# callmeray/PointMVSNet

Hardware: AMD Instinct MI355X
Metric: depth-maps/sec (DTU 640x512, 3 src views, 2 flow iters) (higher is better)
Workload: dtype f32

## Files before the change

### pointmvsnet_amd/csrc/conv3d.hip

```cpp
#include <stdlib.h>

#include "pf_common.h"
#include "pf_bn_resolve.h"

namespace {

typedef float f32x4 __attribute__((ext_vector_type(4)));

struct ConvGeom {
  int Cin, Cout, Di, Hi, Wi, Do, Ho, Wo;
  int ID, IH, IW, IWP, plane;
  int tiles_d, tiles_h, tiles_w;
  int aff_mode, sps, aff_off;
  const float* in_scale;
  const float* in_shift;
  pf_bn_job in_bn;
};

template <int STRIDE, int TD>
struct Stage {
  static constexpr int ID = (TD - 1) * STRIDE + 3;
  static constexpr int IH = 3 * STRIDE + 3;
  static constexpr int IW = 15 * STRIDE + 3;
  static constexpr int IWP = IW + 1;
  static constexpr int RAW = ID * IH * IWP;
  static constexpr int WANT = STRIDE == 1 ? 16 : 17;
  static constexpr int PLANE = RAW + ((WANT - RAW % 32) + 32) % 32;
  static constexpr int ELEMS = ID * IH * IW;
  static constexpr int NXR = (ELEMS + 63) / 64;
};

template <int NT, int STRIDE, int TD, int MINW>
__global__ __launch_bounds__(256, MINW) void conv3d_k3_kernel(const float* __restrict__ x, const float* __restrict__ wp,
                                                        float* __restrict__ y, ConvGeom g,
                                                        double* __restrict__ partials) {
  using St = Stage<STRIDE, TD>;
  constexpr int ID = St::ID, IH = St::IH, IW = St::IW, IWP = St::IWP, PLANE = St::PLANE;
  constexpr int ELEMS = St::ELEMS, NXR = St::NXR;
  constexpr int NCP = NT * 16;
  constexpr int WSZ = 27 * 4 * NCP;
  constexpr int NWR = (WSZ + 255) / 256;
  constexpr int XS = 4 * PLANE;
  extern __shared__ __attribute__((aligned(16))) float lds[];
  float* xs0 = lds;
  float* ws0 = lds + 2 * XS;
  float* tile = lds;
  double* red = reinterpret_cast<double*>(tile + 4 * NCP * 17 + ((4 * NCP * 17) & 1));

  const int tid = threadIdx.x;
  const int wave = __builtin_amdgcn_readfirstlane(tid >> 6), lane = tid & 63;
  const int li = lane & 15, lk = lane >> 4;
  unsigned xb_, xn_;
  pf_xcd_xy<PF_XCD_CONV3D>(xb_, xn_);
  const int n = (int)xn_, bx = (int)xb_;
  const int plane_i = g.Hi * g.Wi, vol_i = plane_i * g.Di;
  const int64_t plane_o = (int64_t)g.Ho * g.Wo, vol_o = plane_o * g.Do;
  const float* xb = x + (int64_t)n * g.Cin * vol_i;
  float* yb = y + (int64_t)n * g.Cout * vol_o;
  const int cgroups = g.Cin >> 2;

  double ssum[NT], ssq[NT];
#pragma unroll
  for (int t = 0; t < NT; ++t) ssum[t] = ssq[t] = 0.0;

  float* aff = lds + g.aff_off;
  if (g.aff_mode == 1) {
    const int stat = n / g.sps;
    for (int e = tid; e < 2 * g.Cin; e += 256)
      aff[e] = e < g.Cin ? g.in_scale[(int64_t)stat * g.Cin + e] : g.in_shift[(int64_t)stat * g.Cin + e - g.Cin];
  } else if (g.aff_mode == 2) {
    pf_bn_resolve<256>(g.in_bn, n / g.sps, aff, aff + g.Cin, reinterpret_cast<double*>(lds));
  }

  const int total = g.tiles_d * g.tiles_h * g.tiles_w;
  for (int item = bx; item < total; item += gridDim.x) {
    const int tw = item % g.tiles_w;
    const int rest = item / g.tiles_w;
    const int th = rest % g.tiles_h;
    const int td = rest / g.tiles_h;
    const int od0 = td * TD, oh0 = th * 4, ow0 = tw * 16;
    const int id0 = od0 * STRIDE - 1, ih0 = oh0 * STRIDE - 1, iw0 = ow0 * STRIDE - 1;

    unsigned gofs[NXR];
    unsigned okmask = 0;
#pragma unroll
    for (int r = 0; r < NXR; ++r) {
      const int e = lane + 64 * r;
      const int row = e / IW, col = e - row * IW;
      const int dz = row / IH, hy = row - dz * IH;
      const int id = id0 + dz, ih = ih0 + hy, iw = iw0 + col;
      const bool ok = e < ELEMS && id >= 0 && id < g.Di && ih >= 0 && ih < g.Hi && iw >= 0 && iw < g.Wi;
      gofs[r] = ok ? (unsigned)(id * plane_i + ih * g.Wi + iw) : 0u;
      okmask |= (ok ? 1u : 0u) << r;
    }

    float rx[NXR], rw[NWR];
    auto load_group = [&](int cg) {
      const float* src = xb + (int64_t)(cg * 4 + wave) * vol_i;
#pragma unroll
      for (int r = 0; r < NXR; ++r) rx[r] = src[gofs[r]];
      const float* wsrc = wp + (int64_t)cg * WSZ;
#pragma unroll
      for (int r = 0; r < NWR; ++r) {
        const int e = tid + 256 * r;
        rw[r] = (256 * (r + 1) <= WSZ || e < WSZ) ? wsrc[e] : 0.0f;
      }
    };
    auto store_group = [&](int buf, int cg) {
      float* xs = xs0 + buf * XS + wave * PLANE;
      float* ws = ws0 + buf * WSZ;
      float sa = 1.0f, sb = 0.0f;
      if (g.aff_mode) {
        sa = aff[cg * 4 + wave];
        sb = aff[g.Cin + cg * 4 + wave];
      }
#pragma unroll
      for (int r = 0; r < NXR; ++r) {
        const int e = lane + 64 * r;
        float v = rx[r];
        if (g.aff_mode) v = fmaxf(fmaf(v, sa, sb), 0.0f);
        if (64 * (r + 1) <= ELEMS || e < ELEMS) xs[e + e / IW] = ((okmask >> r) & 1u) ? v : 0.0f;
      }
#pragma unroll
      for (int r = 0; r < NWR; ++r) {
        const int e = tid + 256 * r;
        if (256 * (r + 1) <= WSZ || e < WSZ) ws[e] = rw[r];
      }
    };

    f32x4 acc[TD][NT];
#pragma unroll
    for (int d = 0; d < TD; ++d)
#pragma unroll
      for (int t = 0; t < NT; ++t) acc[d][t] = (f32x4){0.0f, 0.0f, 0.0f, 0.0f};

    __syncthreads();
    load_group(0);
    store_group(0, 0);
    __syncthreads();
    for (int cg = 0; cg < cgroups; ++cg) {
      const int buf = cg & 1;
      if (cg + 1 < cgroups) load_group(cg + 1);
      const float* xs = xs0 + buf * XS + lk * PLANE + (wave * STRIDE) * IWP + li * STRIDE;
      const float* ws = ws0 + buf * WSZ + lk * NCP + li;
#pragma unroll
      for (int kd = 0; kd < 3; ++kd) {
#pragma unroll
        for (int kh = 0; kh < 3; ++kh) {
#pragma unroll
          for (int kw = 0; kw < 3; ++kw) {
            const int tap = (kd * 3 + kh) * 3 + kw;
            float b[NT];
#pragma unroll
            for (int t = 0; t < NT; ++t) b[t] = ws[tap * 4 * NCP + 16 * t];
#pragma unroll
            for (int d = 0; d < TD; ++d) {
              const float a = xs[((d * STRIDE + kd) * IH + kh) * IWP + kw];
#pragma unroll
              for (int t = 0; t < NT; ++t) acc[d][t] = __builtin_amdgcn_mfma_f32_16x16x4f32(a, b[t], acc[d][t], 0, 0, 0);
            }
          }
        }
      }
      if (cg + 1 < cgroups) store_group(buf ^ 1, cg + 1);
      __syncthreads();
    }

    const int oh = oh0 + wave;
    float* tl = tile + wave * NCP * 17;
#pragma unroll
    for (int d = 0; d < TD; ++d) {
      const int od = od0 + d;
      const bool row_ok = oh < g.Ho && od < g.Do;
#pragma unroll
      for (int t = 0; t < NT; ++t) {
        float s = 0.0f, q = 0.0f;
#pragma unroll
        for (int r = 0; r < 4; ++r) {
          const int pos = lk * 4 + r;
          const float v = acc[d][t][r];
          tl[(16 * t + li) * 17 + pos] = v;
          if (row_ok && ow0 + pos < g.Wo) {
            s += v;
            q += v * v;
          }
        }
        s += __shfl_xor(s, 16);
        q += __shfl_xor(q, 16);
        s += __shfl_xor(s, 32);
        q += __shfl_xor(q, 32);
        ssum[t] += (double)s;
        ssq[t] += (double)q;
      }
      __builtin_amdgcn_wave_barrier();
      if (row_ok) {
        for (int e = lane; e < NCP * 16; e += 64) {
          const int co = e >> 4, pos = e & 15;
          if (co < g.Cout && ow0 + pos < g.Wo)
            yb[(int64_t)co * vol_o + (int64_t)od * plane_o + (int64_t)oh * g.Wo + ow0 + pos] = tl[co * 17 + pos];
        }
      }
      __builtin_amdgcn_wave_barrier();
    }
  }

  if (partials != nullptr) {
#pragma unroll
    for (int t = 0; t < NT; ++t) {
      if (lane < 16) {
        red[((wave * NCP) + 16 * t + lane) * 2 + 0] = ssum[t];
        red[((wave * NCP) + 16 * t + lane) * 2 + 1] = ssq[t];
      }
    }
    __syncthreads();
    if (tid < g.Cout) {
      double s = 0.0, q = 0.0;
#pragma unroll
      for (int w = 0; w < 4; ++w) {
        s += red[((w * NCP) + tid) * 2 + 0];
        q += red[((w * NCP) + tid) * 2 + 1];
      }
      double* o = partials + (((int64_t)n * gridDim.x + bx) * g.Cout + tid) * 2;
      o[0] = s;
      o[1] = q;
    }
  }
}

template <int COUT>
__global__ __launch_bounds__(256) void conv3d_k3_few_kernel(const float* __restrict__ x, const float* __restrict__ w,
                                                            float* __restrict__ y, int Cin, int D, int H, int W) {
  extern __shared__ __attribute__((aligned(16))) float wl[];
  for (int e = threadIdx.x; e < COUT * Cin * 27; e += 256) wl[e] = w[e];
  __syncthreads();
  const int64_t plane = (int64_t)H * W, vol = plane * D;
  const int64_t i = (int64_t)blockIdx.x * 256 + threadIdx.x;
  const int n = blockIdx.y;
  if (i >= vol) return;
  const int od = (int)(i / plane);
  const int rem = (int)(i - (int64_t)od * plane);
  const int oh = rem / W, ow = rem - oh * W;
  float acc[COUT];
#pragma unroll
  for (int c = 0; c < COUT; ++c) acc[c] = 0.0f;
  const float* xb = x + (int64_t)n * Cin * vol;
  for (int ci = 0; ci < Cin; ++ci) {
    const float* xc = xb + (int64_t)ci * vol;
#pragma unroll
    for (int kd = 0; kd < 3; ++kd) {
      const int id = od + kd - 1;
      const bool dok = id >= 0 && id < D;
#pragma unroll
      for (int kh = 0; kh < 3; ++kh) {
        const int ih = oh + kh - 1;
        const bool hok = dok && ih >= 0 && ih < H;
        const float* row = xc + (int64_t)id * plane + (int64_t)ih * W;
#pragma unroll
        for (int kw = 0; kw < 3; ++kw) {
          const int iw = ow + kw - 1;
          const float v = (hok && iw >= 0 && iw < W) ? row[iw] : 0.0f;
#pragma unroll
          for (int c = 0; c < COUT; ++c) acc[c] = fmaf(v, wl[(c * Cin + ci) * 27 + (kd * 3 + kh) * 3 + kw], acc[c]);
        }
      }
    }
  }
#pragma unroll
  for (int c = 0; c < COUT; ++c) y[((int64_t)n * COUT + c) * vol + i] = acc[c];
}

ConvGeom make_geom(int64_t Cin, int64_t Cout, int64_t Di, int64_t Hi, int64_t Wi, int stride, int td) {
  ConvGeom g;
  g.Cin = (int)Cin;
  g.Cout = (int)Cout;
  g.Di = (int)Di;
  g.Hi = (int)Hi;
  g.Wi = (int)Wi;
  g.Do = (int)((Di - 1) / stride + 1);
  g.Ho = (int)((Hi - 1) / stride + 1);
  g.Wo = (int)((Wi - 1) / stride + 1);
  g.ID = (td - 1) * stride + 3;
  g.IH = 3 * stride + 3;
  g.IW = 15 * stride + 3;
  g.IWP = g.IW + 1;
  const int raw = g.ID * g.IH * g.IWP;
  const int want = stride == 1 ? 16 : 17;
  g.plane = raw + ((want - raw % 32) + 32) % 32;
  g.tiles_d = (g.Do + td - 1) / td;
  g.tiles_h = (g.Ho + 3) / 4;
  g.tiles_w = (g.Wo + 15) / 16;
  g.aff_mode = 0;
  g.sps = 1;
  g.aff_off = 0;
  g.in_scale = g.in_shift = nullptr;
  g.in_bn = pf_bn_job{};
  return g;
}

constexpr size_t kMaxLds = 80 * 1024;

size_t lds_work_bytes(const ConvGeom& g, int NT) {
  const int NCP = NT * 16;
  const size_t staging = sizeof(float) * (size_t)(2 * 4 * g.plane + 2 * 27 * 4 * NCP);
  const size_t epilogue = sizeof(float) * (size_t)(4 * NCP * 17 + 1) + sizeof(double) * (size_t)(4 * NCP * 2);
  const size_t m = staging > epilogue ? staging : epilogue;
  return (m + 15) / 16 * 16;
}
size_t lds_bytes_for(const ConvGeom& g, int NT) {
  return lds_work_bytes(g, NT) + sizeof(float) * 2 * (size_t)g.Cin;
}

int pick_td(int64_t Cin, int64_t Cout, int64_t Di, int64_t Hi, int64_t Wi, int stride) {
  const int NT = (int)((Cout + 15) / 16);
  int best = 0;
  for (int td = (stride == 1 && NT > 1) ? 4 : 2; td >= 1; td >>= 1) {
    const ConvGeom g = make_geom(Cin, Cout, Di, Hi, Wi, stride, td);
    if (lds_bytes_for(g, NT) > kMaxLds) continue;
    best = td;
    if ((int64_t)g.tiles_d * g.tiles_h * g.tiles_w >= 512) return td;
  }
  return best;
}

int blocks_for(const ConvGeom& g) {
  const int64_t total = (int64_t)g.tiles_d * g.tiles_h * g.tiles_w;
#ifndef PF_CONV3D_CAP
#define PF_CONV3D_CAP 2048
#endif
  if (total <= PF_CONV3D_CAP) return (int)total;
  const int64_t per = (total + PF_CONV3D_CAP - 1) / PF_CONV3D_CAP;
  return (int)((total + per - 1) / per);
}

template <int NT, int STRIDE, int TD, int MINW>
int launch(const float* x, const float* wp, float* y, const ConvGeom& g, int64_t N, double* partials,
           hipStream_t s) {
  const size_t lds_bytes = lds_bytes_for(g, NT);
  if (lds_bytes > kMaxLds) return PF_ERR_UNSUPPORTED;
  ConvGeom gk = g;
  gk.aff_off = (int)(lds_work_bytes(g, NT) / sizeof(float));
  if (lds_bytes > 64 * 1024) {
    static std::atomic<unsigned long long> done{0};
    const int rc = pf_allow_big_lds(reinterpret_cast<const void*>(&conv3d_k3_kernel<NT, STRIDE, TD, MINW>),
                                    (int)kMaxLds, done);
    if (rc != PF_OK) return rc;
  }
  dim3 grid((unsigned)blocks_for(g), (unsigned)N);
  hipLaunchKernelGGL((conv3d_k3_kernel<NT, STRIDE, TD, MINW>), grid, dim3(256), lds_bytes, s, x, wp, y, gk, partials);
  return pf_launch_status();
}

template <int NT, int STRIDE, int TD>
int launch_w(const float* x, const float* wp, float* y, const ConvGeom& g, int64_t N, double* partials,
             hipStream_t s) {
  constexpr int kDefault = (NT == 1 && STRIDE == 1 && TD == 2) ? 4 : 2;
  return launch<NT, STRIDE, TD, kDefault>(x, wp, y, g, N, partials, s);
}

template <int NT, int STRIDE>
int launch_td(int td, const float* x, const float* wp, float* y, const ConvGeom& g, int64_t N, double* partials,
              hipStream_t s) {
  if constexpr (STRIDE == 1) {
    if (td == 4) return launch_w<NT, STRIDE, 4>(x, wp, y, g, N, partials, s);
  }
  if (td == 2) return launch_w<NT, STRIDE, 2>(x, wp, y, g, N, partials, s);
  return launch_w<NT, STRIDE, 1>(x, wp, y, g, N, partials, s);
}

}

extern "C" {

int pf_conv3d_blocks(int64_t Cin, int64_t Cout, int64_t Di, int64_t Hi, int64_t Wi, int stride) {
  if (Cin <= 0 || Cout <= 0 || Di <= 0 || Hi <= 0 || Wi <= 0 || (stride != 1 && stride != 2)) return 0;
  const int td = pick_td(Cin, Cout, Di, Hi, Wi, stride);
  if (td == 0) return 0;
  return blocks_for(make_geom(Cin, Cout, Di, Hi, Wi, stride, td));
}

int pf_conv3d_k3_f32(const float* x, const float* wp, float* y, int64_t N, int64_t Cin, int64_t Cout, int64_t Di,
                     int64_t Hi, int64_t Wi, int stride, const float* in_scale, const float* in_shift,
                     const pf_bn_job* in_bn, int samples_per_stat, double* partials, void* stream) {
  PF_REQUIRE(N >= 0 && Cin >= 4 && Cout >= 1 && Di >= 1 && Hi >= 1 && Wi >= 1 && N <= 65535);
  PF_REQUIRE(stride == 1 || stride == 2);
  PF_REQUIRE(samples_per_stat >= 1 && (in_scale == nullptr) == (in_shift == nullptr));
  PF_REQUIRE(in_bn == nullptr || in_scale == nullptr);
  if (in_bn != nullptr && N > 0) {
    PF_REQUIRE(N % samples_per_stat == 0);
    const int rc = pf_bn_in_check(in_bn, (int)Cin, (int)(N / samples_per_stat));
    if (rc != PF_OK) return rc;
  }
  if ((Cin % 4) != 0 || Cout > 32) return PF_ERR_UNSUPPORTED;
  PF_REQUIRE(Cin * Di * Hi * Wi <= INT32_MAX);
  if (N == 0) return PF_OK;
  PF_REQUIRE(x && wp && y);
  const int td = pick_td(Cin, Cout, Di, Hi, Wi, stride);
  if (td == 0) return PF_ERR_UNSUPPORTED;
  ConvGeom g = make_geom(Cin, Cout, Di, Hi, Wi, stride, td);
  g.aff_mode = in_bn ? 2 : (in_scale ? 1 : 0);
  g.sps = samples_per_stat;
  g.in_scale = in_scale;
  g.in_shift = in_shift;
  if (in_bn) g.in_bn = *in_bn;
  hipStream_t s = (hipStream_t)stream;
  const int NT = (int)((Cout + 15) / 16);
  if (stride == 1)
    return NT == 1 ? launch_td<1, 1>(td, x, wp, y, g, N, partials, s) : launch_td<2, 1>(td, x, wp, y, g, N, partials, s);
  return NT == 1 ? launch_td<1, 2>(td, x, wp, y, g, N, partials, s) : launch_td<2, 2>(td, x, wp, y, g, N, partials, s);
}

int pf_conv3d_k3_few_f32(const float* x, const float* w, float* y, int64_t N, int64_t Cin, int64_t Cout, int64_t D,
                         int64_t H, int64_t W, void* stream) {
  PF_REQUIRE(N >= 0 && Cin >= 1 && Cout >= 1 && D >= 1 && H >= 1 && W >= 1 && N <= 65535);
  if (Cout > 4 || Cout * Cin * 27 * sizeof(float) > 48 * 1024) return PF_ERR_UNSUPPORTED;
  PF_REQUIRE(H * W <= INT32_MAX);
  if (N == 0) return PF_OK;
  PF_REQUIRE(x && w && y);
  const size_t lds = sizeof(float) * (size_t)(Cout * Cin * 27);
  dim3 grid((unsigned)pf_cdiv(D * H * W, 256), (unsigned)N);
  hipStream_t s = (hipStream_t)stream;
  switch ((int)Cout) {
    case 1: hipLaunchKernelGGL(conv3d_k3_few_kernel<1>, grid, dim3(256), lds, s, x, w, y, (int)Cin, (int)D, (int)H, (int)W); break;
    case 2: hipLaunchKernelGGL(conv3d_k3_few_kernel<2>, grid, dim3(256), lds, s, x, w, y, (int)Cin, (int)D, (int)H, (int)W); break;
    case 3: hipLaunchKernelGGL(conv3d_k3_few_kernel<3>, grid, dim3(256), lds, s, x, w, y, (int)Cin, (int)D, (int)H, (int)W); break;
    default: hipLaunchKernelGGL(conv3d_k3_few_kernel<4>, grid, dim3(256), lds, s, x, w, y, (int)Cin, (int)D, (int)H, (int)W); break;
  }
  return pf_launch_status();
}

}
```

### pointmvsnet_amd/csrc/conv3d_pair.hip

```cpp
#include <stdlib.h>

#include "pf_common.h"

namespace {

typedef float f32x4 __attribute__((ext_vector_type(4)));

struct PairGeom {
  int Cin, Cout, D, H, W;
  int tiles_d, tiles_h, tiles_w;
};

template <int TD>
struct PStage {
  static constexpr int ID = TD + 2;
  static constexpr int IH = 10;
  static constexpr int IW = 18;
  static constexpr int IWP = IW + 1;
  static constexpr int RAW = ID * IH * IWP;
  static constexpr int PLANE = RAW + ((16 - RAW % 32) + 32) % 32;
  static constexpr int ELEMS = ID * IH * IW;
  static constexpr int NXR = (ELEMS + 63) / 64;
};

constexpr int kTaps = 36;
constexpr int kWsz = kTaps * 4 * 16;

template <int TD>
constexpr size_t pair_lds_bytes() {
  using St = PStage<TD>;
  const size_t staging = sizeof(float) * (size_t)(2 * 4 * St::PLANE + 2 * kWsz);
  const size_t epilogue = sizeof(float) * (size_t)(4 * 16 * 17 + 1) + sizeof(double) * (size_t)(4 * 16 * 2);
  return staging > epilogue ? staging : epilogue;
}

template <int TD, int MINW>
__global__ __launch_bounds__(256, MINW) void conv3d_k3_pair_kernel(const float* __restrict__ x,
                                                                   const float* __restrict__ wp,
                                                                   float* __restrict__ y, PairGeom g,
                                                                   double* __restrict__ partials) {
  using St = PStage<TD>;
  constexpr int ID = St::ID, IH = St::IH, IW = St::IW, IWP = St::IWP, PLANE = St::PLANE;
  constexpr int ELEMS = St::ELEMS, NXR = St::NXR;
  constexpr int NWR = (kWsz + 255) / 256;
  constexpr int XS = 4 * PLANE;
  extern __shared__ __attribute__((aligned(16))) float lds[];
  float* xs0 = lds;
  float* ws0 = lds + 2 * XS;
  float* tile = lds;
  double* red = reinterpret_cast<double*>(tile + 4 * 16 * 17 + ((4 * 16 * 17) & 1));

  const int tid = threadIdx.x;
  const int wave = __builtin_amdgcn_readfirstlane(tid >> 6), lane = tid & 63;
  const int li = lane & 15, lk = lane >> 4;
  unsigned xb_, xn_;
  pf_xcd_xy<PF_XCD_CONV3D>(xb_, xn_);
  const int n = (int)xn_, bx = (int)xb_;
  const int plane_i = g.H * g.W, vol = plane_i * g.D;
  const float* xb = x + (int64_t)n * g.Cin * vol;
  float* yb = y + (int64_t)n * g.Cout * vol;
  const int cgroups = g.Cin >> 2;

  double ssum = 0.0, ssq = 0.0;

  const int total = g.tiles_d * g.tiles_h * g.tiles_w;
  for (int item = bx; item < total; item += gridDim.x) {
    const int tw = item % g.tiles_w;
    const int rest = item / g.tiles_w;
    const int th = rest % g.tiles_h;
    const int td = rest / g.tiles_h;
    const int od0 = td * TD, oh0 = th * 8, ow0 = tw * 16;
    const int id0 = od0 - 1, ih0 = oh0 - 1, iw0 = ow0 - 1;

    unsigned gofs[NXR];
    unsigned okmask = 0;
#pragma unroll
    for (int r = 0; r < NXR; ++r) {
      const int e = lane + 64 * r;
      const int row = e / IW, col = e - row * IW;
      const int dz = row / IH, hy = row - dz * IH;
      const int id = id0 + dz, ih = ih0 + hy, iw = iw0 + col;
      const bool ok = e < ELEMS && id >= 0 && id < g.D && ih >= 0 && ih < g.H && iw >= 0 && iw < g.W;
      gofs[r] = ok ? (unsigned)(id * plane_i + ih * g.W + iw) : 0u;
      okmask |= (ok ? 1u : 0u) << r;
    }

    float rx[NXR], rw[NWR];
    auto load_group = [&](int cg) {
      const float* src = xb + (int64_t)(cg * 4 + wave) * vol;
#pragma unroll
      for (int r = 0; r < NXR; ++r) rx[r] = src[gofs[r]];
      const float* wsrc = wp + (int64_t)cg * kWsz;
#pragma unroll
      for (int r = 0; r < NWR; ++r) {
        const int e = tid + 256 * r;
        rw[r] = (256 * (r + 1) <= kWsz || e < kWsz) ? wsrc[e] : 0.0f;
      }
    };
    auto store_group = [&](int buf) {
      float* xs = xs0 + buf * XS + wave * PLANE;
      float* ws = ws0 + buf * kWsz;
#pragma unroll
      for (int r = 0; r < NXR; ++r) {
        const int e = lane + 64 * r;
        if (64 * (r + 1) <= ELEMS || e < ELEMS) xs[e + e / IW] = ((okmask >> r) & 1u) ? rx[r] : 0.0f;
      }
#pragma unroll
      for (int r = 0; r < NWR; ++r) {
        const int e = tid + 256 * r;
        if (256 * (r + 1) <= kWsz || e < kWsz) ws[e] = rw[r];
      }
    };

    f32x4 acc[TD];
#pragma unroll
    for (int d = 0; d < TD; ++d) acc[d] = (f32x4){0.0f, 0.0f, 0.0f, 0.0f};

    __syncthreads();
    load_group(0);
    store_group(0);
    __syncthreads();
    for (int cg = 0; cg < cgroups; ++cg) {
      const int buf = cg & 1;
      if (cg + 1 < cgroups) load_group(cg + 1);
      const float* xs = xs0 + buf * XS + lk * PLANE + (2 * wave) * IWP + li;
      const float* ws = ws0 + buf * kWsz + lk * 16 + li;
#pragma unroll
      for (int kd = 0; kd < 3; ++kd) {
#pragma unroll
        for (int kh = 0; kh < 4; ++kh) {
#pragma unroll
          for (int kw = 0; kw < 3; ++kw) {
            const int tap = (kd * 4 + kh) * 3 + kw;
            const float b = ws[tap * 4 * 16];
#pragma unroll
            for (int d = 0; d < TD; ++d) {
              const float a = xs[((d + kd) * IH + kh) * IWP + kw];
              acc[d] = __builtin_amdgcn_mfma_f32_16x16x4f32(a, b, acc[d], 0, 0, 0);
            }
          }
        }
      }
      if (cg + 1 < cgroups) store_group(buf ^ 1);
      __syncthreads();
    }

    const int oh = oh0 + 2 * wave + (li >> 3);
    float* tl = tile + wave * 16 * 17;
#pragma unroll
    for (int d = 0; d < TD; ++d) {
      const int od = od0 + d;
      const bool row_ok = oh < g.H && od < g.D;
      float s = 0.0f, q = 0.0f;
#pragma unroll
      for (int r = 0; r < 4; ++r) {
        const int pos = lk * 4 + r;
        const float v = acc[d][r];
        tl[li * 17 + pos] = v;
        if (row_ok && ow0 + pos < g.W) {
          s += v;
          q += v * v;
        }
      }
      s += __shfl_xor(s, 8);
      q += __shfl_xor(q, 8);
      s += __shfl_xor(s, 16);
      q += __shfl_xor(q, 16);
      s += __shfl_xor(s, 32);
      q += __shfl_xor(q, 32);
      ssum += (double)s;
      ssq += (double)q;
      __builtin_amdgcn_wave_barrier();
      if (od < g.D) {
        for (int e = lane; e < 16 * 16; e += 64) {
          const int col = e >> 4, pos = e & 15;
          const int co = col & 7, ohh = oh0 + 2 * wave + (col >> 3);
          if (co < g.Cout && ohh < g.H && ow0 + pos < g.W)
            yb[(int64_t)co * vol + (int64_t)od * plane_i + (int64_t)ohh * g.W + ow0 + pos] = tl[col * 17 + pos];
        }
      }
      __builtin_amdgcn_wave_barrier();
    }
  }

  if (partials != nullptr) {
    if (lane < 8) {
      red[(wave * 16 + lane) * 2 + 0] = ssum;
      red[(wave * 16 + lane) * 2 + 1] = ssq;
    }
    __syncthreads();
    if (tid < g.Cout) {
      double s = 0.0, q = 0.0;
#pragma unroll
      for (int w = 0; w < 4; ++w) {
        s += red[(w * 16 + tid) * 2 + 0];
        q += red[(w * 16 + tid) * 2 + 1];
      }
      double* o = partials + (((int64_t)n * gridDim.x + bx) * g.Cout + tid) * 2;
      o[0] = s;
      o[1] = q;
    }
  }
}

#ifndef PF_PAIR_TD
#define PF_PAIR_TD 2
#endif
#ifndef PF_PAIR_MINW
#define PF_PAIR_MINW 3
#endif
constexpr int kPairTD = PF_PAIR_TD;

PairGeom make_pair_geom(int64_t Cin, int64_t Cout, int64_t D, int64_t H, int64_t W) {
  PairGeom g;
  g.Cin = (int)Cin;
  g.Cout = (int)Cout;
  g.D = (int)D;
  g.H = (int)H;
  g.W = (int)W;
  g.tiles_d = (g.D + kPairTD - 1) / kPairTD;
  g.tiles_h = (g.H + 7) / 8;
  g.tiles_w = (g.W + 15) / 16;
  return g;
}

int pair_blocks(const PairGeom& g) {
  const int64_t total = (int64_t)g.tiles_d * g.tiles_h * g.tiles_w;
#ifndef PF_CONV3D_CAP
#define PF_CONV3D_CAP 2048
#endif
  if (total <= PF_CONV3D_CAP) return (int)total;
  const int64_t per = (total + PF_CONV3D_CAP - 1) / PF_CONV3D_CAP;
  return (int)((total + per - 1) / per);
}

}

extern "C" {

int pf_conv3d_pair_blocks(int64_t Cin, int64_t Cout, int64_t D, int64_t H, int64_t W) {
  if (Cin <= 0 || Cout <= 0 || Cout > 8 || D <= 0 || H <= 0 || W <= 0) return 0;
  return pair_blocks(make_pair_geom(Cin, Cout, D, H, W));
}

int pf_conv3d_k3_pair_f32(const float* x, const float* wp, float* y, int64_t N, int64_t Cin, int64_t Cout, int64_t D,
                          int64_t H, int64_t W, double* partials, void* stream) {
  PF_REQUIRE(N >= 0 && Cin >= 4 && Cout >= 1 && D >= 1 && H >= 1 && W >= 1 && N <= 65535);
  if ((Cin % 4) != 0 || Cout > 8) return PF_ERR_UNSUPPORTED;
  PF_REQUIRE(Cin * D * H * W <= INT32_MAX);
  if (N == 0) return PF_OK;
  PF_REQUIRE(x && wp && y);
  const PairGeom g = make_pair_geom(Cin, Cout, D, H, W);
  constexpr size_t lds_bytes = pair_lds_bytes<kPairTD>();
  static_assert(lds_bytes <= 64 * 1024, "pair tile must fit the default dynamic LDS limit");
  dim3 grid((unsigned)pair_blocks(g), (unsigned)N);
  hipLaunchKernelGGL((conv3d_k3_pair_kernel<kPairTD, PF_PAIR_MINW>), grid, dim3(256), lds_bytes, (hipStream_t)stream, x, wp, y, g,
                     partials);
  return pf_launch_status();
}

}
```

### pointmvsnet_amd/csrc/pf_common.h

```cpp
#pragma once

#include <hip/hip_runtime.h>
#include <stdint.h>

#include "pointflow_hip.h"

#define PF_WAVE 64

unsigned* pf_status_ptr();

#define PF_REQUIRE(cond)                 \
  do {                                   \
    if (!(cond)) return PF_ERR_INVALID_ARG; \
  } while (0)

#define PF_HIP(expr)                        \
  do {                                      \
    hipError_t _e = (expr);                 \
    if (_e != hipSuccess) return (int)_e;   \
  } while (0)

static inline int pf_launch_status() {
  hipError_t e = hipGetLastError();
  return e == hipSuccess ? PF_OK : (int)e;
}

static inline int64_t pf_cdiv(int64_t a, int64_t b) { return (a + b - 1) / b; }

#include <atomic>
static inline int pf_allow_big_lds(const void* kernel, int bytes, std::atomic<unsigned long long>& flags) {
  int dev = 0;
  PF_HIP(hipGetDevice(&dev));
  const unsigned long long bit = 1ull << (dev & 63);
  if (flags.load(std::memory_order_acquire) & bit) return PF_OK;
  PF_HIP(hipFuncSetAttribute(kernel, hipFuncAttributeMaxDynamicSharedMemorySize, bytes));
  flags.fetch_or(bit, std::memory_order_release);
  return PF_OK;
}

#if defined(__HIPCC__)
static __global__ __launch_bounds__(256) void pf_zero_kernel(unsigned* __restrict__ p, size_t words) {
  const size_t stride = (size_t)gridDim.x * 256;
  for (size_t i = (size_t)blockIdx.x * 256 + threadIdx.x; i < words; i += stride) p[i] = 0u;
}
static inline int pf_zero_async(void* p, size_t bytes, hipStream_t s) {
  if (bytes == 0) return PF_OK;
  const size_t words = bytes / 4;
  size_t blocks = (words + 255) / 256;
  if (blocks > 4096) blocks = 4096;
  hipLaunchKernelGGL(pf_zero_kernel, dim3((unsigned)blocks), dim3(256), 0, s, reinterpret_cast<unsigned*>(p), words);
  const hipError_t e = hipGetLastError();
  return e == hipSuccess ? PF_OK : (int)e;
}
#endif

#ifndef PF_XCD
#define PF_XCD 1
#endif
#define PF_XCD_TOWER 1
#define PF_XCD_CONV3D 2
#define PF_XCD_FETCH 4
#define PF_XCD_KNN 8
#define PF_XCD_EDGE 16
#define PF_XCD_FRUSTUM 32
#ifdef __HIPCC__
__device__ __forceinline__ unsigned pf_xcd_chunk(unsigned lin, unsigned total) {
  const unsigned per = total >> 3, rem = total & 7u;
  const unsigned x = lin & 7u, j = lin >> 3;
  return x * per + (x < rem ? x : rem) + j;
}
__device__ __forceinline__ unsigned pf_xcd_band(unsigned b, unsigned tiles_per_plane) {
  if ((tiles_per_plane & 7u) != 0u) return b;
  const unsigned band = tiles_per_plane >> 3;
  const unsigned x = b & 7u, j = b >> 3;
  const unsigned d = j / band, o = j - d * band;
  return d * tiles_per_plane + x * band + o;
}
template <int FAMILY>
__device__ __forceinline__ void pf_xcd_xy(unsigned& bx, unsigned& by) {
  if ((PF_XCD & FAMILY) == 0) {
    bx = blockIdx.x;
    by = blockIdx.y;
    return;
  }
  const unsigned gx = gridDim.x;
  const unsigned L = pf_xcd_chunk(blockIdx.y * gx + blockIdx.x, gx * gridDim.y);
  by = L / gx;
  bx = L - by * gx;
}
#endif

struct PfTaps {
  int off[4];
  float wgt[4];
  bool ok[4];
  int xi, yi;
  float fx, fy;
};

__device__ __forceinline__ void pf_project_taps(float X, float Y, float Z, const float* __restrict__ Kv,
                                                const float* __restrict__ Ev, int H, int W, PfTaps& t) {
  float px = X, py = Y, pz = Z;
  if (Ev != nullptr) {
    px = fmaf(Ev[2], Z, fmaf(Ev[1], Y, Ev[0] * X)) + Ev[3];
    py = fmaf(Ev[6], Z, fmaf(Ev[5], Y, Ev[4] * X)) + Ev[7];
    pz = fmaf(Ev[10], Z, fmaf(Ev[9], Y, Ev[8] * X)) + Ev[11];
  }
  const float nx = px / pz;
  const float ny = py / pz;
  const float u = fmaf(Kv[2], 1.0f, fmaf(Kv[1], ny, Kv[0] * nx));
  const float v = fmaf(Kv[5], 1.0f, fmaf(Kv[4], ny, Kv[3] * nx));
  const float gx = ((u - 0.5f) / (float)(W - 1)) * 2.0f - 1.0f;
  const float gy = ((v - 0.5f) / (float)(H - 1)) * 2.0f - 1.0f;
  const float ix = (gx + 1.0f) * ((float)(W - 1) / 2.0f);
  const float iy = (gy + 1.0f) * ((float)(H - 1) / 2.0f);
  const float x0 = floorf(ix), y0 = floorf(iy);
  const float wx1 = ix - x0, wy1 = iy - y0;
  const float wx0 = 1.0f - wx1, wy0 = 1.0f - wy1;
  const float xmax = (float)(W - 1), ymax = (float)(H - 1);
  const bool vx0 = (x0 >= 0.0f) && (x0 <= xmax);
  const bool vx1 = (x0 + 1.0f >= 0.0f) && (x0 + 1.0f <= xmax);
  const bool vy0 = (y0 >= 0.0f) && (y0 <= ymax);
  const bool vy1 = (y0 + 1.0f >= 0.0f) && (y0 + 1.0f <= ymax);
  const int xi = (vx0 || vx1) ? (int)x0 : 0;
  const int yi = (vy0 || vy1) ? (int)y0 : 0;
  t.xi = xi;
  t.yi = yi;
  t.fx = wx1;
  t.fy = wy1;
  t.ok[0] = vy0 && vx0;
  t.ok[1] = vy0 && vx1;
  t.ok[2] = vy1 && vx0;
  t.ok[3] = vy1 && vx1;
  t.off[0] = t.ok[0] ? yi * W + xi : 0;
  t.off[1] = t.ok[1] ? yi * W + xi + 1 : 0;
  t.off[2] = t.ok[2] ? (yi + 1) * W + xi : 0;
  t.off[3] = t.ok[3] ? (yi + 1) * W + xi + 1 : 0;
  t.wgt[0] = t.ok[0] ? wy0 * wx0 : 0.0f;
  t.wgt[1] = t.ok[1] ? wy0 * wx1 : 0.0f;
  t.wgt[2] = t.ok[2] ? wy1 * wx0 : 0.0f;
  t.wgt[3] = t.ok[3] ? wy1 * wx1 : 0.0f;
}

__device__ __forceinline__ float pf_sample(const float* __restrict__ plane, const PfTaps& t) {
  const float a = plane[t.off[0]];
  const float b = plane[t.off[1]];
  const float c = plane[t.off[2]];
  const float d = plane[t.off[3]];
  return ((a * t.wgt[0] + b * t.wgt[1]) + c * t.wgt[2]) + d * t.wgt[3];
}

__device__ __forceinline__ float pf_flow_confidence(const float* __restrict__ prob, int i, int hw) {
  float p[5];
#pragma unroll
  for (int d = 0; d < 5; ++d) p[d] = prob[(int64_t)d * hw + i];
  const double a0 = (double)p[0] * -2.0, a1 = (double)p[1] * -1.0, a2 = (double)p[2] * 0.0;
  const double a3 = (double)p[3] * 1.0, a4 = (double)p[4] * 2.0;
  const double idx = (a0 + (((a1 + a2) + a3) + a4)) + 2.0;
  int fl = (int)floor(idx);
  int ce = fl + 1;
  ce = ce < 0 ? 0 : (ce > 4 ? 4 : ce);
  fl = fl < 0 ? fl + 5 : fl;
  fl = fl < 0 ? 0 : (fl > 4 ? 4 : fl);
  return p[fl] + p[ce];
}
```

Measured before the change: 1089.

## Add narrow conv3d tile widths and single-buffer pair-conv weights with register-pipelined taps

The generic 3x3x3 conv kernel gains a tile-width template parameter (16, 8 or 4 columns with proportionally more rows), chosen per layer to reduce padded area on small outputs. The paired conv kernel single-buffers its weights in LDS to free shared memory and raises minimum waves per SIMD from 3 to 4. Its tap loop is flattened into a software-pipelined sequence that prefetches activations two steps ahead, and address registers are pinned with empty asm. The trade-offs are more template instantiations, an extra barrier per channel group in the pair kernel, and a redundant final load.

Result: no change. 1109, median of 3 (+1.8%).

```diff
diff --git a/pointmvsnet_amd/csrc/conv3d.hip b/pointmvsnet_amd/csrc/conv3d.hip
--- a/pointmvsnet_amd/csrc/conv3d.hip
+++ b/pointmvsnet_amd/csrc/conv3d.hip
@@ -17,25 +17,36 @@
   pf_bn_job in_bn;
 };
 
-template <int STRIDE, int TD>
+constexpr int stage_iw(int stride, int cw) { return (cw - 1) * stride + 3; }
+constexpr int stage_ih(int stride, int cw) { return (64 / cw - 1) * stride + 3; }
+constexpr int stage_iwp(int stride, int cw) {
+  return cw == 16 ? stage_iw(stride, cw) + 1 : cw == 8 ? (stride == 1 ? 16 : 24) : 8;
+}
+constexpr int stage_plane(int stride, int td, int cw) {
+  const int raw = ((td - 1) * stride + 3) * stage_ih(stride, cw) * stage_iwp(stride, cw);
+  const int want = stride == 2 ? 17 : cw;
+  return raw + ((want - raw % 32) + 32) % 32;
+}
+
+template <int STRIDE, int TD, int CW>
 struct Stage {
+  static_assert(CW == 16 || CW == 8 || (CW == 4 && STRIDE == 1), "tile width");
   static constexpr int ID = (TD - 1) * STRIDE + 3;
-  static constexpr int IH = 3 * STRIDE + 3;
-  static constexpr int IW = 15 * STRIDE + 3;
-  static constexpr int IWP = IW + 1;
-  static constexpr int RAW = ID * IH * IWP;
-  static constexpr int WANT = STRIDE == 1 ? 16 : 17;
-  static constexpr int PLANE = RAW + ((WANT - RAW % 32) + 32) % 32;
+  static constexpr int IH = stage_ih(STRIDE, CW);
+  static constexpr int IW = stage_iw(STRIDE, CW);
+  static constexpr int IWP = stage_iwp(STRIDE, CW);
+  static constexpr int PLANE = stage_plane(STRIDE, TD, CW);
   static constexpr int ELEMS = ID * IH * IW;
   static constexpr int NXR = (ELEMS + 63) / 64;
 };
 
-template <int NT, int STRIDE, int TD, int MINW>
+template <int NT, int STRIDE, int TD, int MINW, int CW>
 __global__ __launch_bounds__(256, MINW) void conv3d_k3_kernel(const float* __restrict__ x, const float* __restrict__ wp,
                                                         float* __restrict__ y, ConvGeom g,
                                                         double* __restrict__ partials) {
-  using St = Stage<STRIDE, TD>;
+  using St = Stage<STRIDE, TD, CW>;
   constexpr int ID = St::ID, IH = St::IH, IW = St::IW, IWP = St::IWP, PLANE = St::PLANE;
+  constexpr int RW = 16 / CW;
   constexpr int ELEMS = St::ELEMS, NXR = St::NXR;
   constexpr int NCP = NT * 16;
   constexpr int WSZ = 27 * 4 * NCP;
@@ -78,7 +89,7 @@
     const int rest = item / g.tiles_w;
     const int th = rest % g.tiles_h;
     const int td = rest / g.tiles_h;
-    const int od0 = td * TD, oh0 = th * 4, ow0 = tw * 16;
+    const int od0 = td * TD, oh0 = th * 4 * RW, ow0 = tw * CW;
     const int id0 = od0 * STRIDE - 1, ih0 = oh0 * STRIDE - 1, iw0 = ow0 * STRIDE - 1;
 
     unsigned gofs[NXR];
@@ -119,7 +130,7 @@
         const int e = lane + 64 * r;
         float v = rx[r];
         if (g.aff_mode) v = fmaxf(fmaf(v, sa, sb), 0.0f);
-        if (64 * (r + 1) <= ELEMS || e < ELEMS) xs[e + e / IW] = ((okmask >> r) & 1u) ? v : 0.0f;
+        if (64 * (r + 1) <= ELEMS || e < ELEMS) xs[e + (e / IW) * (IWP - IW)] = ((okmask >> r) & 1u) ? v : 0.0f;
       }
 #pragma unroll
       for (int r = 0; r < NWR; ++r) {
@@ -141,7 +152,7 @@
     for (int cg = 0; cg < cgroups; ++cg) {
       const int buf = cg & 1;
       if (cg + 1 < cgroups) load_group(cg + 1);
-      const float* xs = xs0 + buf * XS + lk * PLANE + (wave * STRIDE) * IWP + li * STRIDE;
+      const float* xs = xs0 + buf * XS + lk * PLANE + ((wave * RW + li / CW) * STRIDE) * IWP + (li % CW) * STRIDE;
       const float* ws = ws0 + buf * WSZ + lk * NCP + li;
 #pragma unroll
       for (int kd = 0; kd < 3; ++kd) {
@@ -166,12 +177,12 @@
       __syncthreads();
     }
 
-    const int oh = oh0 + wave;
+    const int ohw = oh0 + wave * RW;
     float* tl = tile + wave * NCP * 17;
 #pragma unroll
     for (int d = 0; d < TD; ++d) {
       const int od = od0 + d;
-      const bool row_ok = oh < g.Ho && od < g.Do;
+      const bool row_ok = (CW < 16 || ohw < g.Ho) && od < g.Do;
 #pragma unroll
       for (int t = 0; t < NT; ++t) {
         float s = 0.0f, q = 0.0f;
@@ -180,7 +191,7 @@
           const int pos = lk * 4 + r;
           const float v = acc[d][t][r];
           tl[(16 * t + li) * 17 + pos] = v;
-          if (row_ok && ow0 + pos < g.Wo) {
+          if (row_ok && (CW == 16 || ohw + pos / CW < g.Ho) && ow0 + pos % CW < g.Wo) {
             s += v;
             q += v * v;
           }
@@ -196,8 +207,9 @@
       if (row_ok) {
         for (int e = lane; e < NCP * 16; e += 64) {
           const int co = e >> 4, pos = e & 15;
-          if (co < g.Cout && ow0 + pos < g.Wo)
-            yb[(int64_t)co * vol_o + (int64_t)od * plane_o + (int64_t)oh * g.Wo + ow0 + pos] = tl[co * 17 + pos];
+          const int oh = ohw + pos / CW;
+          if (co < g.Cout && (CW == 16 || oh < g.Ho) && ow0 + pos % CW < g.Wo)
+            yb[(int64_t)co * vol_o + (int64_t)od * plane_o + (int64_t)oh * g.Wo + ow0 + pos % CW] = tl[co * 17 + pos];
         }
       }
       __builtin_amdgcn_wave_barrier();
@@ -269,7 +281,7 @@
   for (int c = 0; c < COUT; ++c) y[((int64_t)n * COUT + c) * vol + i] = acc[c];
 }
 
-ConvGeom make_geom(int64_t Cin, int64_t Cout, int64_t Di, int64_t Hi, int64_t Wi, int stride, int td) {
+ConvGeom make_geom(int64_t Cin, int64_t Cout, int64_t Di, int64_t Hi, int64_t Wi, int stride, int td, int cw) {
   ConvGeom g;
   g.Cin = (int)Cin;
   g.Cout = (int)Cout;
@@ -280,15 +292,13 @@
   g.Ho = (int)((Hi - 1) / stride + 1);
   g.Wo = (int)((Wi - 1) / stride + 1);
   g.ID = (td - 1) * stride + 3;
-  g.IH = 3 * stride + 3;
-  g.IW = 15 * stride + 3;
-  g.IWP = g.IW + 1;
-  const int raw = g.ID * g.IH * g.IWP;
-  const int want = stride == 1 ? 16 : 17;
-  g.plane = raw + ((want - raw % 32) + 32) % 32;
+  g.IH = stage_ih(stride, cw);
+  g.IW = stage_iw(stride, cw);
+  g.IWP = stage_iwp(stride, cw);
+  g.plane = stage_plane(stride, td, cw);
   g.tiles_d = (g.Do + td - 1) / td;
-  g.tiles_h = (g.Ho + 3) / 4;
-  g.tiles_w = (g.Wo + 15) / 16;
+  g.tiles_h = (g.Ho + 64 / cw - 1) / (64 / cw);
+  g.tiles_w = (g.Wo + cw - 1) / cw;
   g.aff_mode = 0;
   g.sps = 1;
   g.aff_off = 0;
@@ -310,14 +320,35 @@
   return lds_work_bytes(g, NT) + sizeof(float) * 2 * (size_t)g.Cin;
 }
 
-int pick_td(int64_t Cin, int64_t Cout, int64_t Di, int64_t Hi, int64_t Wi, int stride) {
+int pick_td(int64_t Cin, int64_t Cout, int64_t Di, int64_t Hi, int64_t Wi, int stride, int cw) {
   const int NT = (int)((Cout + 15) / 16);
   int best = 0;
-  for (int td = (stride == 1 && NT > 1) ? 4 : 2; td >= 1; td >>= 1) {
-    const ConvGeom g = make_geom(Cin, Cout, Di, Hi, Wi, stride, td);
+  for (int td = (stride == 2 && cw < 16) ? 1 : (stride == 1 && NT > 1) ? 4 : 2; td >= 1; td >>= 1) {
+    const ConvGeom g = make_geom(Cin, Cout, Di, Hi, Wi, stride, td, cw);
     if (lds_bytes_for(g, NT) > kMaxLds) continue;
     best = td;
     if ((int64_t)g.tiles_d * g.tiles_h * g.tiles_w >= 512) return td;
+  }
+  return best;
+}
+
+int pick_cw(int64_t Cin, int64_t Cout, int64_t Di, int64_t Hi, int64_t Wi, int stride) {
+  const int64_t Ho = (Hi - 1) / stride + 1, Wo = (Wi - 1) / stride + 1;
+  int best = 16;
+  int64_t best_area = 0;
+  for (int cw = 16; cw >= (stride == 1 ? 4 : 8); cw >>= 1) {
+    const int bh = 64 / cw;
+    const int64_t area = (Ho + bh - 1) / bh * bh * ((Wo + cw - 1) / cw * cw);
+    if (cw == 16 || area < best_area) {
+      best = cw;
+      best_area = area;
+    }
+  }
+  if (stride == 2 && best < 16) {
+    const int td = pick_td(Cin, Cout, Di, Hi, Wi, stride, best);
+    if (td == 0) return 16;
+    const ConvGeom g = make_geom(Cin, Cout, Di, Hi, Wi, stride, td, best);
+    if ((int64_t)g.tiles_d * g.tiles_h * g.tiles_w < 256) return 16;
   }
   return best;
 }
@@ -332,7 +363,7 @@
   return (int)((total + per - 1) / per);
 }
 
-template <int NT, int STRIDE, int TD, int MINW>
+template <int NT, int STRIDE, int TD, int MINW, int CW>
 int launch(const float* x, const float* wp, float* y, const ConvGeom& g, int64_t N, double* partials,
            hipStream_t s) {
   const size_t lds_bytes = lds_bytes_for(g, NT);
@@ -341,30 +372,42 @@
   gk.aff_off = (int)(lds_work_bytes(g, NT) / sizeof(float));
   if (lds_bytes > 64 * 1024) {
     static std::atomic<unsigned long long> done{0};
-    const int rc = pf_allow_big_lds(reinterpret_cast<const void*>(&conv3d_k3_kernel<NT, STRIDE, TD, MINW>),
+    const int rc = pf_allow_big_lds(reinterpret_cast<const void*>(&conv3d_k3_kernel<NT, STRIDE, TD, MINW, CW>),
                                     (int)kMaxLds, done);
     if (rc != PF_OK) return rc;
   }
   dim3 grid((unsigned)blocks_for(g), (unsigned)N);
-  hipLaunchKernelGGL((conv3d_k3_kernel<NT, STRIDE, TD, MINW>), grid, dim3(256), lds_bytes, s, x, wp, y, gk, partials);
+  hipLaunchKernelGGL((conv3d_k3_kernel<NT, STRIDE, TD, MINW, CW>), grid, dim3(256), lds_bytes, s, x, wp, y, gk, partials);
   return pf_launch_status();
 }
 
-template <int NT, int STRIDE, int TD>
+template <int NT, int STRIDE, int TD, int CW>
 int launch_w(const float* x, const float* wp, float* y, const ConvGeom& g, int64_t N, double* partials,
              hipStream_t s) {
   constexpr int kDefault = (NT == 1 && STRIDE == 1 && TD == 2) ? 4 : 2;
-  return launch<NT, STRIDE, TD, kDefault>(x, wp, y, g, N, partials, s);
-}
-
-template <int NT, int STRIDE>
+  return launch<NT, STRIDE, TD, kDefault, CW>(x, wp, y, g, N, partials, s);
+}
+
+template <int NT, int STRIDE, int CW>
 int launch_td(int td, const float* x, const float* wp, float* y, const ConvGeom& g, int64_t N, double* partials,
               hipStream_t s) {
   if constexpr (STRIDE == 1) {
-    if (td == 4) return launch_w<NT, STRIDE, 4>(x, wp, y, g, N, partials, s);
-  }
-  if (td == 2) return launch_w<NT, STRIDE, 2>(x, wp, y, g, N, partials, s);
-  return launch_w<NT, STRIDE, 1>(x, wp, y, g, N, partials, s);
+    if (td == 4) return launch_w<NT, STRIDE, 4, CW>(x, wp, y, g, N, partials, s);
+  }
+  if constexpr (STRIDE == 1 || CW == 16) {
+    if (td == 2) return launch_w<NT, STRIDE, 2, CW>(x, wp, y, g, N, partials, s);
+  }
+  return launch_w<NT, STRIDE, 1, CW>(x, wp, y, g, N, partials, s);
+}
+
+template <int NT, int STRIDE>
+int launch_cw(int cw, int td, const float* x, const float* wp, float* y, const ConvGeom& g, int64_t N, double* partials,
+              hipStream_t s) {
+  if (cw == 8) return launch_td<NT, STRIDE, 8>(td, x, wp, y, g, N, partials, s);
+  if constexpr (STRIDE == 1) {
+    if (cw == 4) return launch_td<NT, STRIDE, 4>(td, x, wp, y, g, N, partials, s);
+  }
+  return launch_td<NT, STRIDE, 16>(td, x, wp, y, g, N, partials, s);
 }
 
 }
@@ -373,9 +416,10 @@
 
 int pf_conv3d_blocks(int64_t Cin, int64_t Cout, int64_t Di, int64_t Hi, int64_t Wi, int stride) {
   if (Cin <= 0 || Cout <= 0 || Di <= 0 || Hi <= 0 || Wi <= 0 || (stride != 1 && stride != 2)) return 0;
-  const int td = pick_td(Cin, Cout, Di, Hi, Wi, stride);
+  const int cw = pick_cw(Cin, Cout, Di, Hi, Wi, stride);
+  const int td = pick_td(Cin, Cout, Di, Hi, Wi, stride, cw);
   if (td == 0) return 0;
-  return blocks_for(make_geom(Cin, Cout, Di, Hi, Wi, stride, td));
+  return blocks_for(make_geom(Cin, Cout, Di, Hi, Wi, stride, td, cw));
 }
 
 int pf_conv3d_k3_f32(const float* x, const float* wp, float* y, int64_t N, int64_t Cin, int64_t Cout, int64_t Di,
@@ -394,9 +438,10 @@
   PF_REQUIRE(Cin * Di * Hi * Wi <= INT32_MAX);
   if (N == 0) return PF_OK;
   PF_REQUIRE(x && wp && y);
-  const int td = pick_td(Cin, Cout, Di, Hi, Wi, stride);
+  const int cw = pick_cw(Cin, Cout, Di, Hi, Wi, stride);
+  const int td = pick_td(Cin, Cout, Di, Hi, Wi, stride, cw);
   if (td == 0) return PF_ERR_UNSUPPORTED;
-  ConvGeom g = make_geom(Cin, Cout, Di, Hi, Wi, stride, td);
+  ConvGeom g = make_geom(Cin, Cout, Di, Hi, Wi, stride, td, cw);
   g.aff_mode = in_bn ? 2 : (in_scale ? 1 : 0);
   g.sps = samples_per_stat;
   g.in_scale = in_scale;
@@ -405,8 +450,10 @@
   hipStream_t s = (hipStream_t)stream;
   const int NT = (int)((Cout + 15) / 16);
   if (stride == 1)
-    return NT == 1 ? launch_td<1, 1>(td, x, wp, y, g, N, partials, s) : launch_td<2, 1>(td, x, wp, y, g, N, partials, s);
-  return NT == 1 ? launch_td<1, 2>(td, x, wp, y, g, N, partials, s) : launch_td<2, 2>(td, x, wp, y, g, N, partials, s);
+    return NT == 1 ? launch_cw<1, 1>(cw, td, x, wp, y, g, N, partials, s)
+                   : launch_cw<2, 1>(cw, td, x, wp, y, g, N, partials, s);
+  return NT == 1 ? launch_cw<1, 2>(cw, td, x, wp, y, g, N, partials, s)
+                 : launch_cw<2, 2>(cw, td, x, wp, y, g, N, partials, s);
 }
 
 int pf_conv3d_k3_few_f32(const float* x, const float* w, float* y, int64_t N, int64_t Cin, int64_t Cout, int64_t D,
diff --git a/pointmvsnet_amd/csrc/conv3d_pair.hip b/pointmvsnet_amd/csrc/conv3d_pair.hip
--- a/pointmvsnet_amd/csrc/conv3d_pair.hip
+++ b/pointmvsnet_amd/csrc/conv3d_pair.hip
@@ -29,7 +29,7 @@
 template <int TD>
 constexpr size_t pair_lds_bytes() {
   using St = PStage<TD>;
-  const size_t staging = sizeof(float) * (size_t)(2 * 4 * St::PLANE + 2 * kWsz);
+  const size_t staging = sizeof(float) * (size_t)(2 * 4 * St::PLANE + kWsz);
   const size_t epilogue = sizeof(float) * (size_t)(4 * 16 * 17 + 1) + sizeof(double) * (size_t)(4 * 16 * 2);
   return staging > epilogue ? staging : epilogue;
 }
@@ -42,7 +42,9 @@
   using St = PStage<TD>;
   constexpr int ID = St::ID, IH = St::IH, IW = St::IW, IWP = St::IWP, PLANE = St::PLANE;
   constexpr int ELEMS = St::ELEMS, NXR = St::NXR;
-  constexpr int NWR = (kWsz + 255) / 256;
+  constexpr int NWR = kWsz / 256;
+  constexpr int kSteps = (TD + 2) * 12;
+  static_assert(kWsz % 256 == 0, "weights of a group: whole rounds of the block");
   constexpr int XS = 4 * PLANE;
   extern __shared__ __attribute__((aligned(16))) float lds[];
   float* xs0 = lds;
@@ -81,35 +83,32 @@
       const int dz = row / IH, hy = row - dz * IH;
       const int id = id0 + dz, ih = ih0 + hy, iw = iw0 + col;
       const bool ok = e < ELEMS && id >= 0 && id < g.D && ih >= 0 && ih < g.H && iw >= 0 && iw < g.W;
-      gofs[r] = ok ? (unsigned)(id * plane_i + ih * g.W + iw) : 0u;
+      gofs[r] = ok ? 4u * (unsigned)(id * plane_i + ih * g.W + iw) : 0u;
       okmask |= (ok ? 1u : 0u) << r;
     }
 
-    float rx[NXR], rw[NWR];
+    float rx[NXR];
+    float rw[NWR];
     auto load_group = [&](int cg) {
-      const float* src = xb + (int64_t)(cg * 4 + wave) * vol;
-#pragma unroll
-      for (int r = 0; r < NXR; ++r) rx[r] = src[gofs[r]];
+      const char* src = reinterpret_cast<const char*>(xb + (int64_t)(cg * 4 + wave) * vol);
+#pragma unroll
+      for (int r = 0; r < NXR; ++r) rx[r] = *reinterpret_cast<const float*>(src + pf_pinned(gofs[r]));
       const float* wsrc = wp + (int64_t)cg * kWsz;
 #pragma unroll
-      for (int r = 0; r < NWR; ++r) {
-        const int e = tid + 256 * r;
-        rw[r] = (256 * (r + 1) <= kWsz || e < kWsz) ? wsrc[e] : 0.0f;
-      }
+      for (int r = 0; r < NWR; ++r) rw[r] = wsrc[tid + 256 * r];
     };
     auto store_group = [&](int buf) {
       float* xs = xs0 + buf * XS + wave * PLANE;
-      float* ws = ws0 + buf * kWsz;
+      const int ln = (int)pf_pinned((unsigned)lane);
 #pragma unroll
       for (int r = 0; r < NXR; ++r) {
-        const int e = lane + 64 * r;
-        if (64 * (r + 1) <= ELEMS || e < ELEMS) xs[e + e / IW] = ((okmask >> r) & 1u) ? rx[r] : 0.0f;
-      }
-#pragma unroll
-      for (int r = 0; r < NWR; ++r) {
-        const int e = tid + 256 * r;
-        if (256 * (r + 1) <= kWsz || e < kWsz) ws[e] = rw[r];
-      }
+        const int e = ln + 64 * r;
+        xs[(64 * (r + 1) <= ELEMS || e < ELEMS) ? e + e / IW : IW] = ((okmask >> r) & 1u) ? rx[r] : 0.0f;
+      }
+    };
+    auto store_weights = [&]() {
+#pragma unroll
+      for (int r = 0; r < NWR; ++r) ws0[tid + 256 * r] = rw[r];
     };
 
     f32x4 acc[TD];
@@ -119,30 +118,36 @@
     __syncthreads();
     load_group(0);
     store_group(0);
+    store_weights();
     __syncthreads();
     for (int cg = 0; cg < cgroups; ++cg) {
       const int buf = cg & 1;
-      if (cg + 1 < cgroups) load_group(cg + 1);
+      load_group(cg + 1 < cgroups ? cg + 1 : cg);
       const float* xs = xs0 + buf * XS + lk * PLANE + (2 * wave) * IWP + li;
-      const float* ws = ws0 + buf * kWsz + lk * 16 + li;
-#pragma unroll
-      for (int kd = 0; kd < 3; ++kd) {
-#pragma unroll
-        for (int kh = 0; kh < 4; ++kh) {
-#pragma unroll
-          for (int kw = 0; kw < 3; ++kw) {
-            const int tap = (kd * 4 + kh) * 3 + kw;
+      const float* ws = ws0 + lk * 16 + li;
+      auto a_at = [&](int s) { return xs[((s / 12) * IH + (s % 12) / 3) * IWP + s % 3]; };
+      float a0 = a_at(0), a1 = a_at(1);
+#pragma unroll
+      for (int s = 0; s < kSteps; ++s) {
+        float a2 = a1;
+        if (s + 2 < kSteps) a2 = a_at(s + 2);
+#pragma unroll
+        for (int d = 0; d < TD; ++d) {
+          const int tap = s - 12 * d;
+          if (tap >= 0 && tap < kTaps) {
             const float b = ws[tap * 4 * 16];
-#pragma unroll
-            for (int d = 0; d < TD; ++d) {
-              const float a = xs[((d + kd) * IH + kh) * IWP + kw];
-              acc[d] = __builtin_amdgcn_mfma_f32_16x16x4f32(a, b, acc[d], 0, 0, 0);
-            }
+            acc[d] = __builtin_amdgcn_mfma_f32_16x16x4f32(a0, b, acc[d], 0, 0, 0);
           }
         }
-      }
-      if (cg + 1 < cgroups) store_group(buf ^ 1);
+        a0 = a1;
+        a1 = a2;
+      }
+      store_group(buf ^ 1);
       __syncthreads();
+      if (cg + 1 < cgroups) {
+        store_weights();
+        __syncthreads();
+      }
     }
 
     const int oh = oh0 + 2 * wave + (li >> 3);
@@ -207,7 +212,7 @@
 #define PF_PAIR_TD 2
 #endif
 #ifndef PF_PAIR_MINW
-#define PF_PAIR_MINW 3
+#define PF_PAIR_MINW 4
 #endif
 constexpr int kPairTD = PF_PAIR_TD;
 
diff --git a/pointmvsnet_amd/csrc/pf_common.h b/pointmvsnet_amd/csrc/pf_common.h
--- a/pointmvsnet_amd/csrc/pf_common.h
+++ b/pointmvsnet_amd/csrc/pf_common.h
@@ -88,6 +88,12 @@
   by = L / gx;
   bx = L - by * gx;
 }
+__device__ __forceinline__ unsigned pf_pinned(unsigned v) {
+#if defined(__HIP_DEVICE_COMPILE__)
+  asm volatile("" : "+v"(v));
+#endif
+  return v;
+}
 #endif
 
 struct PfTaps {
```
